# fengranMark/HAConvDR

Measured on AMD Instinct MI355X. Metric: queries/sec (encode+top-100) over N-passage 768-d corpus; HBM GB/s vs peak, higher is better.
Workload: dtype bf16 MFMA operands with fp32 accumulate / LayerNorm / softmax in the encoder (cosine vs the fp32 reference within 1e-3, measured ~1e-5); search scores and order = the fp32 fmaf chain, bit-exact

## Files before the change

haconvdr_amd/csrc/gemm8.inc:

```

enum { EPI8_QKV = 0, EPI8_RESID = 2, EPI8_GELU = 3 };
#ifndef G8_N1
#define G8_N1 4
#endif

struct Gemm8Args {
    const bf16 *A;
    const bf16 *W;
    int N, K;
    int n_groups;
    int n_tile0;
    const int *total_rows;
    const float2 *astats;
    const float *wsum;
    const float *cvec;
    bf16 *q, *k, *v16;
    const bf16 *resid;
    const float2 *rstats;
    const float *rgamma, *rbeta;
    bf16 *yb;
    float2 *part;
    bf16 *h;
    unsigned long long *clk;
    int stagger;
    int stagger_mode;
};

__device__ __forceinline__ void glds16(const bf16 *src, unsigned char *dst) {
    typedef const __attribute__((address_space(1))) void *gvp;
    typedef __attribute__((address_space(3))) void *lvp;
    __builtin_amdgcn_global_load_lds((gvp)src, (lvp)dst, 16, 0, 0);
}
__device__ __forceinline__ void swap16(unsigned &a, unsigned &b) {
    const auto r = __builtin_amdgcn_permlane16_swap(a, b, false, false);
    a = r[0];
    b = r[1];
}
__device__ __forceinline__ void quad_transpose4(f4v &v, int p) {
    int x0 = __float_as_int(v.x), x1 = __float_as_int(v.y), x2 = __float_as_int(v.z), x3 = __float_as_int(v.w);
    {
        const bool odd = p & 1;
        const int sa = odd ? x0 : x1, sb = odd ? x2 : x3;
        const int ra = __builtin_amdgcn_update_dpp(0, sa, 0xB1, 0xF, 0xF, false);
        const int rb = __builtin_amdgcn_update_dpp(0, sb, 0xB1, 0xF, 0xF, false);
        x0 = odd ? ra : x0;
        x1 = odd ? x1 : ra;
        x2 = odd ? rb : x2;
        x3 = odd ? x3 : rb;
    }
    {
        const bool hi = p & 2;
        const int sa = hi ? x0 : x2, sb = hi ? x1 : x3;
        const int ra = __builtin_amdgcn_update_dpp(0, sa, 0x4E, 0xF, 0xF, false);
        const int rb = __builtin_amdgcn_update_dpp(0, sb, 0x4E, 0xF, 0xF, false);
        x0 = hi ? ra : x0;
        x2 = hi ? x2 : ra;
        x1 = hi ? rb : x1;
        x3 = hi ? x3 : rb;
    }
    v.x = __int_as_float(x0);
    v.y = __int_as_float(x1);
    v.z = __int_as_float(x2);
    v.w = __int_as_float(x3);
}

__device__ __forceinline__ void xchg8(uint4 &a, uint4 &b, bool lo) {
    unsigned *pa = reinterpret_cast<unsigned *>(&a), *pb = reinterpret_cast<unsigned *>(&b);
#pragma unroll
    for (int i = 0; i < 4; ++i) {
        const unsigned send = lo ? pb[i] : pa[i];
        const unsigned recv = (unsigned)__builtin_amdgcn_update_dpp(0, (int)send, 0x128, 0xF, 0xF, false);
        pa[i] = lo ? pa[i] : recv;
        pb[i] = lo ? recv : pb[i];
    }
}

typedef unsigned g8_u4 __attribute__((ext_vector_type(4)));
typedef unsigned g8_u2 __attribute__((ext_vector_type(2)));
template <bool NT> __device__ __forceinline__ void g8_store16(void *p, uint4 v) {
    if constexpr (NT) __builtin_nontemporal_store(g8_u4{v.x, v.y, v.z, v.w}, reinterpret_cast<g8_u4 *>(p));
    else *reinterpret_cast<uint4 *>(p) = v;
}
template <bool NT> __device__ __forceinline__ void g8_store8(void *p, uint2 v) {
    if constexpr (NT) __builtin_nontemporal_store(g8_u2{v.x, v.y}, reinterpret_cast<g8_u2 *>(p));
    else *reinterpret_cast<uint2 *>(p) = v;
}

__device__ __forceinline__ unsigned pack_bf16(float lo, float hi) {
    typedef __bf16 bf16x2_t __attribute__((ext_vector_type(2)));
    bf16x2_t v;
    v.x = (bf16)lo;
    v.y = (bf16)hi;
    return __builtin_bit_cast(unsigned, v);
}

__device__ __forceinline__ f2v gelu8_2(f2v x) {
    f2v z = x * 0.70710678118654752f;
    z.x = __builtin_amdgcn_fmed3f(z.x, -3.0f, 3.0f);
    z.y = __builtin_amdgcn_fmed3f(z.y, -3.0f, 3.0f);
    const f2v u = z * z;
    f2v p = u * (-1.546677965e-07f) + 6.9032217e-06f;
    p = p * u + (-0.0001336812065f);
    p = p * u + 0.001487465865f;
    p = p * u + (-0.0106578986f);
    p = p * u + 0.0524059485f;
    p = p * u + (-0.1851637965f);
    p = p * u + 0.56346134f;
    return x * (z * p + 0.5f);
}

template <int EPI, bool NT>
__global__ __launch_bounds__(512, 2) void gemm8_kernel(Gemm8Args g) {
    extern __shared__ __attribute__((aligned(16))) unsigned char smem[];
    const int tid = threadIdx.x, lane = tid & 63;
    const int w = __builtin_amdgcn_readfirstlane(tid >> 6);
    const int wr = w >> 2, wc = w & 3;
    if constexpr (EPI == EPI8_GELU) {
        if (g.clk && blockIdx.x == 0 && tid == 0) {
            g.clk[0] = __builtin_amdgcn_s_memtime();
            g.clk[1] = __builtin_amdgcn_s_memrealtime();
        }
    }
    const int K = g.K, KT = K >> 6, nx = (g.N >> 8) - g.n_tile0;
    const int NG = g.n_groups, nxg = nx / NG, NP = 8 / NG;
    const int xcd = blockIdx.x & 7, slot = blockIdx.x >> 3, per_xcd = (gridDim.x + 7 - xcd) >> 3;
    const int mt_all = (*g.total_rows + 255) >> 8;
    const int mt_lo = (int)((long)mt_all * (xcd / NG) / NP), mt_hi = (int)((long)mt_all * (xcd / NG + 1) / NP);
    const int n_base = g.n_tile0 + (xcd % NG) * nxg;
    const int run_lo = 0, run_hi = (mt_hi - mt_lo) * nxg;
    const int tile0 = run_lo + slot;
    if (tile0 >= run_hi) return;
    const int my_tiles = (run_hi - tile0 + per_xcd - 1) / per_xcd;
    const int srow = lane >> 3;
    const int sch0 = (lane & 7) ^ (srow >> 1);
    const int chE = sch0 * 8, chO = (sch0 ^ 4) * 8;
    int s_tile = tile0, s_kt = 0;
    const bf16 *s_A = g.A + (size_t)((mt_lo + s_tile / nxg) << 8) * K, *s_W = g.W + (size_t)((n_base + s_tile % nxg) << 8) * K;
    const int wq = w & 3;
    const int so = EPI == EPI8_RESID ? wr : wr ^ 1;
    const unsigned lsrcE = (unsigned)(((so ? wq * 64 : wq * 32) + srow) * K + chE);
    const unsigned lsrcO = (unsigned)(((so ? wq * 64 : wq * 32) + 8 + srow) * K + chO);
    const int ring_base = (so ? 98304 : 0) + wq * 4096, ring_slots = so ? 4 : 6;
    int h_half = 0, h_slot = 0, h_p = 0;
    const bf16 *h_base = so ? s_W : s_A;
    long h_left = (long)my_tiles * KT * 8;
    constexpr int N1 = G8_N1, N2 = 8 - N1;
    auto issue_piece = [&]() __attribute__((always_inline)) {
        const bf16 *src = h_base + (size_t)(h_half * (so ? 32 : 128) + (h_p >> 1) * 16) * K + s_kt * 64;
        unsigned char *dst = smem + ring_base + (h_slot << 14) + h_p * 1024;
        glds16(src + ((h_p & 1) ? lsrcO : lsrcE), dst);
        if (++h_p == 4) {
            h_p = 0;
            h_slot = h_slot + 1 == ring_slots ? 0 : h_slot + 1;
            if (++h_half == 2) {
                h_half = 0;
                if (++s_kt == KT) {
                    s_kt = 0;
                    s_tile += per_xcd;
                    h_base = so ? g.W + (size_t)((n_base + s_tile % nxg) << 8) * K : g.A + (size_t)((mt_lo + s_tile / nxg) << 8) * K;
                }
            }
        }
    };
    auto issue_pieces = [&](auto ntag) __attribute__((always_inline)) -> bool {
        constexpr int n = decltype(ntag)::value;
        if (h_left <= 0) return false;
        h_left -= n;
#pragma unroll
        for (int i = 0; i < n; ++i) issue_piece();
        return true;
    };
    constexpr std::integral_constant<int, 16> n16tag{};
    constexpr std::integral_constant<int, 8> n8ktag{};

    const int m16 = lane & 15, kg = lane >> 4, sw = (m16 >> 1) & 7;
    const int c0 = ((kg ^ sw) << 4), c1 = (((4 + kg) ^ sw) << 4);
    const int a_row = (wr * 64 + m16) * 128, w_row = (wc * 32 + m16) * 128;

#ifdef G8_STAMP
    unsigned long long stamps[16] = {0, 0, 0, 0, 0, 0, 0, 0, 0, 0, 0, 0, 0, 0, 0, 0};
    unsigned long long est[16] = {0, 0, 0, 0, 0, 0, 0, 0, 0, 0, 0, 0, 0, 0, 0, 0};
#define G8_T(i, cond) if (cond) stamps[i] = __builtin_amdgcn_s_memtime()
#define G8_E(i) if (seq == 2) est[i] = __builtin_amdgcn_s_memtime()
#else
#define G8_E(i)
#define G8_T(i, cond)
#endif
#ifdef G8_STAMP2
    unsigned long long ph[16] = {0, 0, 0, 0, 0, 0, 0, 0, 0, 0, 0, 0, 0, 0, 0, 0};
#define G8_P(i) if (seq == 3 && kt == 6) ph[i] = __builtin_amdgcn_s_memtime()
#define G8_PM() if (seq == 3 && kt == 6) ph[5] = ph[6] = ph[13] = ph[7] = ph[8] = ph[9] = __builtin_amdgcn_s_memtime()
#else
#define G8_P(i)
#define G8_PM()
#endif
    constexpr bool RL = EPI == EPI8_RESID;
    f32x4 acc[2][2][4][2];
    bf16x8 wf0[2][2], wf1[2][2], af0[4][2];

    issue_pieces(n16tag);
    if (g.stagger) {
        const int ph = g.stagger_mode == 0 ? (xcd & 3) : g.stagger_mode == 1 ? (slot & 3) : g.stagger_mode == 2 ? xcd : (slot & 7);
        for (int i = ph * g.stagger; i > 0; --i) __builtin_amdgcn_s_sleep(32);
    }
    asm volatile("s_waitcnt vmcnt(0)" ::: "memory");
    __builtin_amdgcn_s_barrier();

    int a_cur = 0, w_cur = 0;
    for (int seq = 0; seq < my_tiles; ++seq) {
        const int tile = tile0 + seq * per_xcd;
        const int m0 = (mt_lo + tile / nxg) << 8, n0 = (n_base + tile % nxg) << 8;
        unsigned char *R1 = smem, *R2 = smem, *R3 = smem;
        const size_t rl_tb = (size_t)m0 * H + n0;
        auto rl_issue_sb = [&](int i, int mt, unsigned char *dst) __attribute__((always_inline)) {
            int ln = lane;
            asm volatile("" : "+v"(ln));
            const unsigned lo = (unsigned)((ln & 15) * H + (ln >> 5) * 16 + ((ln >> 4) & 1) * 8);
#if defined(G8_RL_ABL) && (G8_RL_ABL & 2)
            const bf16 *src = g.resid + (size_t)(wr * 64 + i * 128 + mt * 16) * H + wc * 64 + lo;
#else
            const bf16 *src = g.resid + (rl_tb + (size_t)(wr * 64 + i * 128 + mt * 16) * H + wc * 64) + lo;
#endif
            glds16(src, dst);
            glds16(src + 32, dst + 1024);
        };
        auto rl_issue_cols = [&](unsigned char *dst) __attribute__((always_inline)) {
            int ln = lane;
            asm volatile("" : "+v"(ln));
            const unsigned so = (unsigned)((ln >> 5) * 128 + 2 * (ln & 31));
            glds16(reinterpret_cast<const bf16 *>(g.rstats + ((size_t)m0 + wr * 64) + so), dst);
            const int sel = (ln >> 4) & 3;
            const float *pc = g.cvec, *pg = g.rgamma, *pb = g.rbeta;
            asm volatile("" : "+s"(pc), "+s"(pg), "+s"(pb));
            const float *vb = pc;
            vb = sel == 1 ? pg : vb;
            vb = sel == 2 ? pb : vb;
            glds16(reinterpret_cast<const bf16 *>(vb + (n0 + wc * 64) + 4 * (ln & 15)), dst + 1024);
        };
        G8_T(2, seq == 3);
        if (wr == 1) __builtin_amdgcn_s_barrier();
#pragma unroll
        for (int i = 0; i < 2; ++i)
#pragma unroll
            for (int j = 0; j < 2; ++j)
#pragma unroll
                for (int mt = 0; mt < 4; ++mt)
#pragma unroll
                    for (int nt = 0; nt < 2; ++nt)
#pragma unroll
                        for (int e = 0; e < 4; ++e) acc[i][j][mt][nt][e] = 0.f;

        for (int kt = 0; kt < KT; ++kt) {
            G8_P(0);
            const unsigned char *kbA = smem + a_cur * 32768, *kbW = smem + 98304 + w_cur * 32768;
            if constexpr (!RL) {
                const bool staged = (wr || kt) && issue_pieces(n8ktag);
                __builtin_amdgcn_sched_barrier(0);
                G8_P(12);
#pragma unroll
                for (int nt = 0; nt < 2; ++nt) {
                    wf0[nt][0] = *reinterpret_cast<const bf16x8 *>(kbW + w_row + nt * 2048 + c0);
                    wf0[nt][1] = *reinterpret_cast<const bf16x8 *>(kbW + w_row + nt * 2048 + c1);
                    wf1[nt][0] = *reinterpret_cast<const bf16x8 *>(kbW + 16384 + w_row + nt * 2048 + c0);
                    wf1[nt][1] = *reinterpret_cast<const bf16x8 *>(kbW + 16384 + w_row + nt * 2048 + c1);
                }
#pragma unroll
                for (int mt = 0; mt < 4; ++mt) {
                    af0[mt][0] = *reinterpret_cast<const bf16x8 *>(kbA + a_row + mt * 2048 + c0);
                    af0[mt][1] = *reinterpret_cast<const bf16x8 *>(kbA + a_row + mt * 2048 + c1);
                }
                __builtin_amdgcn_sched_barrier(0);
                G8_P(1);
                G8_P(2);
                if (wr && kt) {
                    if (staged) asm volatile("s_waitcnt vmcnt(8)" ::: "memory");
                    else asm volatile("s_waitcnt vmcnt(0)" ::: "memory");
                }
                asm volatile("s_waitcnt lgkmcnt(0)" ::: "memory");
                G8_P(3);
                __builtin_amdgcn_s_barrier();
                G8_P(4);
                G8_T(3 + (kt < 3 ? kt : 3), seq == 3 && kt < 4);
                __builtin_amdgcn_sched_barrier(0);
                __builtin_amdgcn_s_setprio(1);
                auto read_a1 = [&](auto mttag, auto kstag) __attribute__((always_inline)) {
                    constexpr int mt = decltype(mttag)::value, ks = decltype(kstag)::value;
                    __builtin_amdgcn_sched_barrier(0);
                    af0[mt][ks] = *reinterpret_cast<const bf16x8 *>(kbA + 16384 + a_row + mt * 2048 + (ks ? c1 : c0));
                    __builtin_amdgcn_sched_barrier(0);
                };
                constexpr std::integral_constant<int, 0> i0{};
                constexpr std::integral_constant<int, 1> i1{};
                constexpr std::integral_constant<int, 2> i2{};
                constexpr std::integral_constant<int, 3> i3{};
                auto mfma4 = [&](auto itag, auto mttag, auto kstag) __attribute__((always_inline)) {
                    constexpr int i = decltype(itag)::value, mt = decltype(mttag)::value, ks = decltype(kstag)::value;
#pragma unroll
                    for (int nt = 0; nt < 2; ++nt) {
                        acc[i][0][mt][nt] = __builtin_amdgcn_mfma_f32_16x16x32_bf16(wf0[nt][ks], af0[mt][ks], acc[i][0][mt][nt], 0, 0, 0);
                        acc[i][1][mt][nt] = __builtin_amdgcn_mfma_f32_16x16x32_bf16(wf1[nt][ks], af0[mt][ks], acc[i][1][mt][nt], 0, 0, 0);
                    }
                };
                mfma4(i0, i0, i0), read_a1(i0, i0);
                mfma4(i0, i1, i0), read_a1(i1, i0);
                mfma4(i0, i2, i0), read_a1(i2, i0);
                mfma4(i0, i3, i0), read_a1(i3, i0);
                mfma4(i0, i0, i1), read_a1(i0, i1);
                mfma4(i0, i1, i1), read_a1(i1, i1);
                mfma4(i0, i2, i1);
                mfma4(i0, i3, i1);
                __builtin_amdgcn_sched_barrier(0);
                G8_PM();
                mfma4(i1, i0, i0), read_a1(i2, i1);
                mfma4(i1, i1, i0), read_a1(i3, i1);
                mfma4(i1, i2, i0);
                mfma4(i1, i3, i0);
                __builtin_amdgcn_sched_barrier(0);
                mfma4(i1, i0, i1);
                mfma4(i1, i1, i1);
                mfma4(i1, i2, i1);
                mfma4(i1, i3, i1);
                __builtin_amdgcn_s_setprio(0);
                G8_P(10);
                if (wr == 0 && kt) asm volatile("s_waitcnt vmcnt(0)" ::: "memory");
                asm volatile("s_waitcnt lgkmcnt(0)" ::: "memory");
                __builtin_amdgcn_s_barrier();
                G8_P(11);
                a_cur = a_cur == 2 ? 0 : a_cur + 1;
                w_cur ^= 1;
                continue;
            }
            const bool lastk = RL && kt == KT - 1;
            const bool live1 = (wr == 0 || kt) && h_left > 0 && !(lastk && wr == 0);
            if (live1) {
                h_left -= N1;
#pragma unroll
                for (int i = 0; i < N1; ++i) issue_piece();
            }
            if constexpr (RL) {
                if (lastk) {
                    R1 = smem + (a_cur == 0 ? 2 : a_cur - 1) * 32768 + w * 4096;
                    R3 = smem + a_cur * 32768 + w * 4096;
                    R2 = smem + 98304 + w_cur * 32768 + w * 4096;
                    rl_issue_cols(R1);
                    rl_issue_sb(0, 0, R1 + 2048);
                }
            }
            __builtin_amdgcn_sched_barrier(0);
            G8_P(12);
#pragma unroll
            for (int nt = 0; nt < 2; ++nt) {
                wf0[nt][0] = *reinterpret_cast<const bf16x8 *>(kbW + w_row + nt * 2048 + c0);
                wf0[nt][1] = *reinterpret_cast<const bf16x8 *>(kbW + w_row + nt * 2048 + c1);
                wf1[nt][0] = *reinterpret_cast<const bf16x8 *>(kbW + 16384 + w_row + nt * 2048 + c0);
                wf1[nt][1] = *reinterpret_cast<const bf16x8 *>(kbW + 16384 + w_row + nt * 2048 + c1);
            }
#pragma unroll
            for (int mt = 0; mt < 4; ++mt) {
                af0[mt][0] = *reinterpret_cast<const bf16x8 *>(kbA + a_row + mt * 2048 + c0);
                af0[mt][1] = *reinterpret_cast<const bf16x8 *>(kbA + a_row + mt * 2048 + c1);
            }
            __builtin_amdgcn_sched_barrier(0);
            G8_P(1);
            G8_P(2);
            asm volatile("s_waitcnt lgkmcnt(0)" ::: "memory");
            G8_P(3);
            __builtin_amdgcn_s_barrier();
            G8_P(4);
            G8_T(3 + (kt < 3 ? kt : 3), seq == 3 && kt < 4);
            __builtin_amdgcn_sched_barrier(0);
            __builtin_amdgcn_s_setprio(1);
#pragma unroll
            for (int ks = 0; ks < 2; ++ks)
#pragma unroll
                for (int mt = 0; mt < 4; ++mt)
#pragma unroll
                    for (int nt = 0; nt < 2; ++nt) {
                        acc[0][0][mt][nt] = __builtin_amdgcn_mfma_f32_16x16x32_bf16(wf0[nt][ks], af0[mt][ks], acc[0][0][mt][nt], 0, 0, 0);
                        acc[0][1][mt][nt] = __builtin_amdgcn_mfma_f32_16x16x32_bf16(wf1[nt][ks], af0[mt][ks], acc[0][1][mt][nt], 0, 0, 0);
                    }
            __builtin_amdgcn_s_setprio(0);
            G8_P(5);
            __builtin_amdgcn_s_barrier();
            G8_P(6);
            const bool live2 = h_left > 0 && !lastk;
            if (live2) {
                h_left -= N2;
#pragma unroll
                for (int i = 0; i < N2; ++i) issue_piece();
            }
            if constexpr (RL) {
                if (lastk) {
                    rl_issue_sb(0, 1, R2);
                    rl_issue_sb(0, 2, R2 + 2048);
                }
            }
            __builtin_amdgcn_sched_barrier(0);
            G8_P(13);
#pragma unroll
            for (int mt = 0; mt < 4; ++mt) {
                af0[mt][0] = *reinterpret_cast<const bf16x8 *>(kbA + 16384 + a_row + mt * 2048 + c0);
                af0[mt][1] = *reinterpret_cast<const bf16x8 *>(kbA + 16384 + a_row + mt * 2048 + c1);
            }
            __builtin_amdgcn_sched_barrier(0);
            G8_P(7);
            if (lastk) {
            } else if (kt) {
                if (!live2) asm volatile("s_waitcnt vmcnt(0)" ::: "memory");
                else if (wr == 0) asm volatile("s_waitcnt vmcnt(8)" ::: "memory");
                else asm volatile("s_waitcnt vmcnt(%0)" ::"n"(N2) : "memory");
            }
            asm volatile("s_waitcnt lgkmcnt(0)" ::: "memory");
            G8_P(8);
            __builtin_amdgcn_s_barrier();
            G8_P(9);
            __builtin_amdgcn_sched_barrier(0);
            __builtin_amdgcn_s_setprio(1);
#pragma unroll
            for (int ks = 0; ks < 2; ++ks)
#pragma unroll
                for (int mt = 0; mt < 4; ++mt)
#pragma unroll
                    for (int nt = 0; nt < 2; ++nt) {
                        acc[1][0][mt][nt] = __builtin_amdgcn_mfma_f32_16x16x32_bf16(wf0[nt][ks], af0[mt][ks], acc[1][0][mt][nt], 0, 0, 0);
                        acc[1][1][mt][nt] = __builtin_amdgcn_mfma_f32_16x16x32_bf16(wf1[nt][ks], af0[mt][ks], acc[1][1][mt][nt], 0, 0, 0);
                    }
            __builtin_amdgcn_s_setprio(0);
            G8_P(10);
            __builtin_amdgcn_s_barrier();
            G8_P(11);
            a_cur = a_cur == 2 ? 0 : a_cur + 1;
            w_cur ^= 1;
        }
        G8_T(8, seq == 2 && true);
        if (wr == 0) __builtin_amdgcn_s_barrier();
        G8_T(0, seq == 2);
        if constexpr (!RL) {
            if (wr == 0) issue_pieces(n8ktag);
            asm volatile("s_waitcnt vmcnt(0)" ::: "memory");
        }
        G8_T(1, seq == 2);

#ifdef G8_NO_EPI
#pragma unroll
        for (int i = 0; i < 2; ++i)
#pragma unroll
            for (int j = 0; j < 2; ++j)
#pragma unroll
                for (int mt = 0; mt < 4; ++mt)
#pragma unroll
                    for (int nt = 0; nt < 2; ++nt) asm volatile("" ::"v"(acc[i][j][mt][nt]));
        continue;
#endif
        {
            const int colg = 8 * ((kg & 1) * 2 + (kg >> 1));
            if constexpr (RL) {
                const bool lo8 = m16 < 8;
                const unsigned lane_b = (unsigned)((wr * 64 + (m16 & 7)) * H + wc * 64 + (m16 >> 3) * 32 + colg);
                const unsigned rd_off = (unsigned)(((kg >> 1) * 16 + m16) * 16);
                const bool rd_hi = kg & 1;
#define G8_VM(n) asm volatile("s_waitcnt vmcnt(" #n ")" ::: "memory")
#define G8_VMC(c, a, b) do { if (c) G8_VM(a); else G8_VM(b); } while (0)
#define G8_LDS_DONE() asm volatile("s_waitcnt lgkmcnt(0)" ::: "memory")
                constexpr std::integral_constant<int, -1> cnone{};
                constexpr std::integral_constant<int, 0> c0t{};
                constexpr std::integral_constant<int, 1> c1t{};
                constexpr std::integral_constant<int, 2> c2t{};
                constexpr std::integral_constant<int, 3> c3t{};
                constexpr std::integral_constant<int, 8> n8tag{};
                rl_issue_sb(0, 3, R3);
                rl_issue_sb(1, 0, R3 + 2048);
                G8_E(0);
                G8_VM(8);
                G8_E(1);
                float mean_[2][4], rstd_[2][4];
                f4v rg[2][2], rb[2][2];
#pragma unroll
                for (int i = 0; i < 2; ++i)
#pragma unroll
                    for (int mt = 0; mt < 4; ++mt) {
                        g8_u4 c = *reinterpret_cast<const g8_u4 *>(R1 + i * 512 + (mt * 16 + (m16 & 14)) * 8);
                        asm volatile("" : "+v"(c));
                        asm volatile("v_mov_b32 %0, %1" : "=v"(mean_[i][mt]) : "v"((m16 & 1) ? c.z : c.x));
                        asm volatile("v_mov_b32 %0, %1" : "=v"(rstd_[i][mt]) : "v"((m16 & 1) ? c.w : c.y));
                    }
#pragma unroll
                for (int jj = 0; jj < 2; ++jj)
#pragma unroll
                    for (int nt = 0; nt < 2; ++nt) {
                        const int co = (jj * 32 + nt * 16 + 4 * kg) * 4;
                        const f4v cvv = *reinterpret_cast<const f4v *>(R1 + 1024 + co);
#pragma unroll
                        for (int i = 0; i < 2; ++i)
#pragma unroll
                            for (int mt = 0; mt < 4; ++mt) acc[i][jj][mt][nt] += cvv;
                        rg[jj][nt] = *reinterpret_cast<const f4v *>(R1 + 1024 + 256 + co);
                        rb[jj][nt] = *reinterpret_cast<const f4v *>(R1 + 1024 + 512 + co);
                    }
                auto sb_read = [&](const unsigned char *sb, g8_u4 (&c)[2][2]) __attribute__((always_inline)) {
#pragma unroll
                    for (int jj = 0; jj < 2; ++jj) {
                        c[jj][0] = *reinterpret_cast<const g8_u4 *>(sb + jj * 1024 + rd_off);
                        c[jj][1] = *reinterpret_cast<const g8_u4 *>(sb + jj * 1024 + 512 + rd_off);
                        asm volatile("" : "+v"(c[jj][0]), "+v"(c[jj][1]));
                    }
                };
                auto sb_do = [&](auto itag, auto mttag, unsigned char *sb, auto refilltag, const g8_u4 (*pre)[2]) __attribute__((always_inline)) {
                    constexpr int i = decltype(itag)::value, mt = decltype(mttag)::value, refill = decltype(refilltag)::value;
                    const float mean = mean_[i][mt], rstd = rstd_[i][mt];
                    uint4 ro[2];
                    float s1 = 0.f, s2 = 0.f;
                    g8_u4 cc[2][2];
                    if (pre) {
#pragma unroll
                        for (int jj = 0; jj < 2; ++jj) cc[jj][0] = pre[jj][0], cc[jj][1] = pre[jj][1];
                    } else {
                        sb_read(sb, cc);
                    }
#pragma unroll
                    for (int jj = 0; jj < 2; ++jj) {
                        const g8_u4 c0 = cc[jj][0], c1 = cc[jj][1];
                        const uint2 w0 = {rd_hi ? c0.z : c0.x, rd_hi ? c0.w : c0.y}, w1 = {rd_hi ? c1.z : c1.x, rd_hi ? c1.w : c1.y};
                        const f4v ra = {__uint_as_float(w0.x << 16), __uint_as_float(w0.x & 0xffff0000u), __uint_as_float(w0.y << 16), __uint_as_float(w0.y & 0xffff0000u)};
                        const f4v rb_ = {__uint_as_float(w1.x << 16), __uint_as_float(w1.x & 0xffff0000u), __uint_as_float(w1.y << 16), __uint_as_float(w1.y & 0xffff0000u)};
                        const f4v o0 = acc[i][jj][mt][0] + ((ra - mean) * rstd * rg[jj][0] + rb[jj][0]);
                        const f4v o1 = acc[i][jj][mt][1] + ((rb_ - mean) * rstd * rg[jj][1] + rb[jj][1]);
                        unsigned p0 = pack_bf16(o0.x, o0.y), p1 = pack_bf16(o0.z, o0.w);
                        unsigned p2 = pack_bf16(o1.x, o1.y), p3 = pack_bf16(o1.z, o1.w);
                        swap16(p0, p2);
                        swap16(p1, p3);
                        ro[jj] = make_uint4(p0, p1, p2, p3);
                        const f4v sm = o0 + o1, sq = o0 * o0 + o1 * o1;
                        const float t1 = (sm.x + sm.y) + (sm.z + sm.w), t2 = (sq.x + sq.y) + (sq.z + sq.w);
                        s1 = jj ? s1 + t1 : t1;
                        s2 = jj ? s2 + t2 : t2;
                    }
                    s1 += __shfl_xor(s1, 16);
                    s2 += __shfl_xor(s2, 16);
                    s1 += __shfl_xor(s1, 32);
                    s2 += __shfl_xor(s2, 32);
                    xchg8(ro[0], ro[1], lo8);
                    G8_LDS_DONE();
                    if constexpr (refill >= 0) rl_issue_sb(1, refill, sb);
                    __builtin_amdgcn_sched_barrier(0);
                    const size_t row = (size_t)m0 + i * 128 + wr * 64 + mt * 16 + m16;
#if defined(G8_RL_ABL) && (G8_RL_ABL & 1)
                    if (lane == 0) g.part[row * (g.N >> 6) + (n0 >> 6) + wc] = make_float2(s1, s2);
#pragma unroll
                    for (int jj = 0; jj < 2; ++jj)
                        if (lane == 0) g8_store16<NT>(g.yb + rl_tb + (size_t)((i * 128 + mt * 16 + jj * 8) * H) + lane_b, ro[jj]);
#else
                    if (kg == 0) g.part[row * (g.N >> 6) + (n0 >> 6) + wc] = make_float2(s1, s2);
#pragma unroll
                    for (int jj = 0; jj < 2; ++jj)
                        g8_store16<NT>(g.yb + rl_tb + (size_t)((i * 128 + mt * 16 + jj * 8) * H) + lane_b, ro[jj]);
#endif
                    __builtin_amdgcn_sched_barrier(0);
                };
                __builtin_amdgcn_sched_barrier(0);
                bool gA = false, gW = false;
                sb_do(c0t, c0t, R1 + 2048, cnone, nullptr);
                G8_E(2);
                __builtin_amdgcn_s_barrier();
                if (wr == 0) gA = issue_pieces(n8tag);
                __builtin_amdgcn_sched_barrier(0);
                G8_E(3);
                G8_VMC(gA, 17, 9);
                G8_E(4);
                sb_do(c0t, c1t, R2, c1t, nullptr);
                G8_VMC(gA, 20, 12);
                G8_E(5);
                sb_do(c0t, c2t, R2 + 2048, c2t, nullptr);
                G8_VMC(gA, 23, 15);
                G8_E(6);
                sb_do(c0t, c3t, R3, c3t, nullptr);
                G8_VMC(gA, 26, 18);
                G8_E(7);
                sb_do(c1t, c0t, R3 + 2048, cnone, nullptr);
                G8_VM(16);
                G8_E(8);
                sb_do(c1t, c1t, R2, cnone, nullptr);
                G8_VM(14);
                G8_E(9);
                sb_do(c1t, c2t, R2 + 2048, cnone, nullptr);
                G8_E(10);
                G8_VM(12);
                G8_E(11);
                g8_u4 c7[2][2];
                sb_read(R3, c7);
                G8_LDS_DONE();
                __builtin_amdgcn_s_barrier();
                if (wr == 1) gW = issue_pieces(n8tag);
                __builtin_amdgcn_sched_barrier(0);
                G8_E(12);
                sb_do(c1t, c3t, R3, cnone, c7);
                G8_E(13);
                G8_VMC(gW, 3, 27);
                G8_E(14);
                G8_E(15);
#undef G8_VM
#undef G8_VMC
#undef G8_LDS_DONE
            } else {
                float2 st[2][4];
#pragma unroll
                for (int i = 0; i < 2; ++i)
#pragma unroll
                    for (int mt = 0; mt < 4; ++mt) st[i][mt] = g.astats[(size_t)m0 + i * 128 + wr * 64 + mt * 16 + m16];
                const int ldo = EPI == EPI8_GELU ? g.N : H;
                const bool lo8 = m16 < 8;
                const unsigned lane_b = (unsigned)((wr * 64 + (m16 & 7)) * ldo + wc * 64 + (m16 >> 3) * 32 + colg);
                f4v ws[2][2], cv[2][2];
#pragma unroll
                for (int j = 0; j < 2; ++j)
#pragma unroll
                    for (int nt = 0; nt < 2; ++nt) {
                        const int nb = n0 + wc * 64 + j * 32;
                        cv[j][nt] = *reinterpret_cast<const f4v *>(g.cvec + nb + nt * 16 + 4 * kg);
                        ws[j][nt] = *reinterpret_cast<const f4v *>(g.wsum + nb + nt * 16 + 4 * kg);
                    }
#pragma unroll
                for (int i = 0; i < 2; ++i)
#pragma unroll
                    for (int mt = 0; mt < 4; ++mt) {
                        const float nm = -st[i][mt].x * st[i][mt].y;
                        float rs = st[i][mt].y;
                        asm volatile("v_mov_b32 %0, %1" : "=v"(rs) : "v"(st[i][mt].y));
                        uint4 o[2];
#pragma unroll
                        for (int j = 0; j < 2; ++j) {
                            const int nb = n0 + wc * 64 + j * 32;
                            unsigned p[4];
#pragma unroll
                            for (int nt = 0; nt < 2; ++nt) {
                                f4v v = acc[i][j][mt][nt] * rs + (ws[j][nt] * nm + cv[j][nt]);
                                if (EPI == EPI8_QKV && n0 >= 2 * H) {
                                    quad_transpose4(v, lane & 3);
                                    const int n = nb + nt * 16 + 4 * kg + (lane & 3) - 2 * H;
                                    const size_t mg = (size_t)(m0 + i * 128 + wr * 64 + mt * 16) >> 4;
                                    uint2 o2;
                                    o2.x = pack_bf16(v.x, v.y);
                                    o2.y = pack_bf16(v.z, v.w);
                                    g8_store8<NT>(g.v16 + (mg * H + n) * 16 + (m16 & 12), o2);
                                    continue;
                                }
                                if constexpr (EPI == EPI8_GELU) {
                                    const f2v g0 = gelu8_2((f2v){v.x, v.y}), g1 = gelu8_2((f2v){v.z, v.w});
                                    p[2 * nt] = pack_bf16(g0.x, g0.y);
                                    p[2 * nt + 1] = pack_bf16(g1.x, g1.y);
                                } else {
                                    p[2 * nt] = pack_bf16(v.x, v.y);
                                    p[2 * nt + 1] = pack_bf16(v.z, v.w);
                                }
                            }
                            if (EPI == EPI8_QKV && n0 >= 2 * H) continue;
                            swap16(p[0], p[2]);
                            swap16(p[1], p[3]);
                            o[j] = make_uint4(p[0], p[1], p[2], p[3]);
                        }
                        if (EPI == EPI8_QKV && n0 >= 2 * H) continue;
                        xchg8(o[0], o[1], lo8);
                        const size_t ur = (size_t)(m0 + i * 128 + mt * 16) * ldo;
#pragma unroll
                        for (int j = 0; j < 2; ++j) {
                            if constexpr (EPI == EPI8_GELU) {
                                g8_store16<NT>(g.h + ur + (size_t)(j * 8) * ldo + n0 + lane_b, o[j]);
                            } else {
                                bf16 *dst = n0 < H ? g.q + ur + n0 : g.k + ur + (n0 - H);
                                g8_store16<NT>(dst + (size_t)(j * 8) * ldo + lane_b, o[j]);
                            }
                        }
                    }
            }
        }
    }
    if constexpr (EPI == EPI8_GELU) {
        if (g.clk && blockIdx.x == 0 && tid == 0) {
            g.clk[2] = __builtin_amdgcn_s_memtime();
            g.clk[3] = __builtin_amdgcn_s_memrealtime();
        }
    }
#ifdef G8_STAMP2
    if (blockIdx.x == 8 && lane == 0 && (w == 0 || w == 4)) {
        unsigned long long *o = reinterpret_cast<unsigned long long *>(g.part) + 64 + (w ? 16 : 0);
        for (int i = 0; i < 16; ++i) o[i] = ph[i];
    }
#endif
#ifdef G8_STAMP
    if (blockIdx.x == 8 && lane == 0 && (w == 0 || w == 4)) {
        unsigned long long *o = reinterpret_cast<unsigned long long *>(g.part) + (w ? 16 : 0);
        for (int i = 0; i < 16; ++i) o[i] = stamps[i];
        for (int i = 0; i < 16; ++i) o[32 + i] = est[i];
    }
#endif
}

__global__ __launch_bounds__(256) void ln_combine_kernel(const float2 *__restrict__ part, int n_part, int n_cols, const int *__restrict__ total_rows,
                                                         float eps, float2 *__restrict__ stats) {
    const size_t row = (size_t)blockIdx.x * 256 + threadIdx.x;
    if (row >= (size_t)((*total_rows + 255) & ~255)) return;
    float s1 = 0.f, s2 = 0.f;
    if ((n_part & 1) == 0) {
        const float4 *p4 = reinterpret_cast<const float4 *>(part + row * n_part);
        float4 v[8];
        const int n4 = n_part >> 1;
#pragma unroll
        for (int i = 0; i < 8; ++i) v[i] = i < n4 ? p4[i] : make_float4(0.f, 0.f, 0.f, 0.f);
#pragma unroll
        for (int i = 0; i < 8; ++i) {
            s1 += v[i].x + v[i].z;
            s2 += v[i].y + v[i].w;
        }
        for (int i = 16; i < n_part; ++i) {
            const float2 p = part[row * n_part + i];
            s1 += p.x;
            s2 += p.y;
        }
    } else {
        for (int i = 0; i < n_part; ++i) {
            const float2 p = part[row * n_part + i];
            s1 += p.x;
            s2 += p.y;
        }
    }
    const float mean = s1 / n_cols;
    const float var = fmaxf(s2 / n_cols - mean * mean, 0.f);
    stats[row] = make_float2(mean, rsqrtf(var + eps));
}

__global__ __launch_bounds__(256) void fold_ln_kernel(const float *__restrict__ Wf, const float *__restrict__ bias, const float *__restrict__ gamma,
                                                      const float *__restrict__ beta, int K, float scale, bf16 *__restrict__ Wb,
                                                      float *__restrict__ wsum, float *__restrict__ cvec) {
    __shared__ float red[2][4];
    const int n = blockIdx.x, tid = threadIdx.x;
    float s = 0.f, c = 0.f;
    for (int k = tid; k < K; k += 256) {
        const float wv = Wf[(size_t)n * K + k];
        const bf16 wb = (bf16)(wv * (gamma ? gamma[k] : 1.f) * scale);
        Wb[(size_t)n * K + k] = wb;
        s += (float)wb;
        if (beta) c += beta[k] * wv;
    }
    s = wave_sum(s);
    c = wave_sum(c);
    if ((tid & 63) == 0) {
        red[0][tid >> 6] = s;
        red[1][tid >> 6] = c;
    }
    __syncthreads();
    if (tid == 0) {
        wsum[n] = gamma ? (red[0][0] + red[0][1]) + (red[0][2] + red[0][3]) : 0.f;
        cvec[n] = (bias[n] + (red[1][0] + red[1][1]) + (red[1][2] + red[1][3])) * scale;
    }
}

__global__ void fill_identity_stats_kernel(float2 *__restrict__ stats, size_t n) {
    const size_t i = (size_t)blockIdx.x * blockDim.x + threadIdx.x;
    if (i < n) stats[i] = make_float2(0.f, 1.f);
}
```

Measured before the change: 8192.

## Swap A/W operand roles for V tiles to drop the quad-transpose epilogue

For QKV tiles in the V range, the loader now swaps which half of the ring receives A and which receives W. The MFMA result therefore comes out already transposed, and the V epilogue can store the transposed bf16 layout directly. This removes the DPP quad_transpose4 shuffles and the scattered 8-byte stores. The per-row stats and wsum/cvec are now loaded along the opposite axes. It also adds timestamp probe macros. The risk is correctness of the role swap and the new index math.

```diff
diff --git a/haconvdr_amd/csrc/gemm8.inc b/haconvdr_amd/csrc/gemm8.inc
--- a/haconvdr_amd/csrc/gemm8.inc
+++ b/haconvdr_amd/csrc/gemm8.inc
@@ -36,34 +36,6 @@
     a = r[0];
     b = r[1];
 }
-__device__ __forceinline__ void quad_transpose4(f4v &v, int p) {
-    int x0 = __float_as_int(v.x), x1 = __float_as_int(v.y), x2 = __float_as_int(v.z), x3 = __float_as_int(v.w);
-    {
-        const bool odd = p & 1;
-        const int sa = odd ? x0 : x1, sb = odd ? x2 : x3;
-        const int ra = __builtin_amdgcn_update_dpp(0, sa, 0xB1, 0xF, 0xF, false);
-        const int rb = __builtin_amdgcn_update_dpp(0, sb, 0xB1, 0xF, 0xF, false);
-        x0 = odd ? ra : x0;
-        x1 = odd ? x1 : ra;
-        x2 = odd ? rb : x2;
-        x3 = odd ? x3 : rb;
-    }
-    {
-        const bool hi = p & 2;
-        const int sa = hi ? x0 : x2, sb = hi ? x1 : x3;
-        const int ra = __builtin_amdgcn_update_dpp(0, sa, 0x4E, 0xF, 0xF, false);
-        const int rb = __builtin_amdgcn_update_dpp(0, sb, 0x4E, 0xF, 0xF, false);
-        x0 = hi ? ra : x0;
-        x2 = hi ? x2 : ra;
-        x1 = hi ? rb : x1;
-        x3 = hi ? x3 : rb;
-    }
-    v.x = __int_as_float(x0);
-    v.y = __int_as_float(x1);
-    v.z = __int_as_float(x2);
-    v.w = __int_as_float(x3);
-}
-
 __device__ __forceinline__ void xchg8(uint4 &a, uint4 &b, bool lo) {
     unsigned *pa = reinterpret_cast<unsigned *>(&a), *pb = reinterpret_cast<unsigned *>(&b);
 #pragma unroll
@@ -143,6 +115,12 @@
     const int ring_base = (so ? 98304 : 0) + wq * 4096, ring_slots = so ? 4 : 6;
     int h_half = 0, h_slot = 0, h_p = 0;
     const bf16 *h_base = so ? s_W : s_A;
+    auto swapped_base = [&](int t) __attribute__((always_inline)) -> const bf16 * {
+        const int nt_ = n_base + t % nxg, mt_ = mt_lo + t / nxg;
+        const bool vt = (nt_ << 8) >= 2 * H;
+        return (so != 0) != vt ? g.W + (size_t)(nt_ << 8) * K : g.A + (size_t)(mt_ << 8) * K;
+    };
+    if constexpr (EPI == EPI8_QKV) h_base = swapped_base(s_tile);
     long h_left = (long)my_tiles * KT * 8;
     constexpr int N1 = G8_N1, N2 = 8 - N1;
     auto issue_piece = [&]() __attribute__((always_inline)) {
@@ -157,7 +135,8 @@
                 if (++s_kt == KT) {
                     s_kt = 0;
                     s_tile += per_xcd;
-                    h_base = so ? g.W + (size_t)((n_base + s_tile % nxg) << 8) * K : g.A + (size_t)((mt_lo + s_tile / nxg) << 8) * K;
+                    if constexpr (EPI == EPI8_QKV) h_base = swapped_base(s_tile);
+                    else h_base = so ? g.W + (size_t)((n_base + s_tile % nxg) << 8) * K : g.A + (size_t)((mt_lo + s_tile / nxg) << 8) * K;
                 }
             }
         }
@@ -182,8 +161,10 @@
     unsigned long long est[16] = {0, 0, 0, 0, 0, 0, 0, 0, 0, 0, 0, 0, 0, 0, 0, 0};
 #define G8_T(i, cond) if (cond) stamps[i] = __builtin_amdgcn_s_memtime()
 #define G8_E(i) if (seq == 2) est[i] = __builtin_amdgcn_s_memtime()
+#define G8_V(i, cond) if (cond) est[i] = __builtin_amdgcn_s_memtime()
 #else
 #define G8_E(i)
+#define G8_V(i, cond)
 #define G8_T(i, cond)
 #endif
 #ifdef G8_STAMP2
@@ -281,6 +262,7 @@
                 __builtin_amdgcn_s_barrier();
                 G8_P(4);
                 G8_T(3 + (kt < 3 ? kt : 3), seq == 3 && kt < 4);
+                G8_V(4, seq == 4 && kt == 0);
                 __builtin_amdgcn_sched_barrier(0);
                 __builtin_amdgcn_s_setprio(1);
                 auto read_a1 = [&](auto mttag, auto kstag) __attribute__((always_inline)) {
@@ -602,6 +584,63 @@
 #undef G8_VMC
 #undef G8_LDS_DONE
             } else {
+                if constexpr (EPI == EPI8_QKV) {
+                    if (n0 >= 2 * H) {
+                        G8_V(2, seq == 3);
+                        f4v rs[2][2], nm[2][2];
+                        float wsf[2][4], cvf[2][4];
+                        float4 sab[2][2][2];
+#pragma unroll
+                        for (int j = 0; j < 2; ++j)
+#pragma unroll
+                            for (int nt = 0; nt < 2; ++nt) {
+                                const float4 *sp = reinterpret_cast<const float4 *>(g.astats + ((size_t)m0 + wc * 64 + j * 32 + nt * 16 + 4 * kg));
+                                sab[j][nt][0] = sp[0];
+                                sab[j][nt][1] = sp[1];
+                            }
+#pragma unroll
+                        for (int i = 0; i < 2; ++i)
+#pragma unroll
+                            for (int mt = 0; mt < 4; ++mt) {
+                                const int n = n0 + i * 128 + wr * 64 + mt * 16 + m16;
+                                wsf[i][mt] = g.wsum[n];
+                                cvf[i][mt] = g.cvec[n];
+                            }
+                        __builtin_amdgcn_sched_barrier(0);
+#pragma unroll
+                        for (int j = 0; j < 2; ++j)
+#pragma unroll
+                            for (int nt = 0; nt < 2; ++nt) {
+                                const float4 sa = sab[j][nt][0], sb = sab[j][nt][1];
+                                float r0, r1, r2, r3;
+                                asm volatile("v_mov_b32 %0, %1" : "=v"(r0) : "v"(sa.y));
+                                asm volatile("v_mov_b32 %0, %1" : "=v"(r1) : "v"(sa.w));
+                                asm volatile("v_mov_b32 %0, %1" : "=v"(r2) : "v"(sb.y));
+                                asm volatile("v_mov_b32 %0, %1" : "=v"(r3) : "v"(sb.w));
+                                rs[j][nt] = (f4v){r0, r1, r2, r3};
+                                nm[j][nt] = (f4v){-sa.x * sa.y, -sa.z * sa.w, -sb.x * sb.y, -sb.z * sb.w};
+                            }
+                        bf16 *vb = g.v16 + ((size_t)((m0 + wc * 64) >> 4) * H + (n0 - 2 * H)) * 16;
+                        const unsigned lane_v = (unsigned)((wr * 64 + m16) * 16 + 4 * kg);
+#pragma unroll
+                        for (int i = 0; i < 2; ++i)
+#pragma unroll
+                            for (int mt = 0; mt < 4; ++mt)
+#pragma unroll
+                                for (int j = 0; j < 2; ++j)
+#pragma unroll
+                                    for (int nt = 0; nt < 2; ++nt) {
+                                        const f4v v = acc[i][j][mt][nt] * rs[j][nt] + (nm[j][nt] * wsf[i][mt] + cvf[i][mt]);
+                                        uint2 o2;
+                                        o2.x = pack_bf16(v.x, v.y);
+                                        o2.y = pack_bf16(v.z, v.w);
+                                        g8_store8<NT>(vb + (size_t)((j * 2 + nt) * H + i * 128 + mt * 16) * 16 + lane_v, o2);
+                                    }
+                        G8_V(3, seq == 3);
+                        continue;
+                    }
+                }
+                G8_V(0, seq == 2);
                 float2 st[2][4];
 #pragma unroll
                 for (int i = 0; i < 2; ++i)
@@ -629,21 +668,10 @@
                         uint4 o[2];
 #pragma unroll
                         for (int j = 0; j < 2; ++j) {
-                            const int nb = n0 + wc * 64 + j * 32;
                             unsigned p[4];
 #pragma unroll
                             for (int nt = 0; nt < 2; ++nt) {
                                 f4v v = acc[i][j][mt][nt] * rs + (ws[j][nt] * nm + cv[j][nt]);
-                                if (EPI == EPI8_QKV && n0 >= 2 * H) {
-                                    quad_transpose4(v, lane & 3);
-                                    const int n = nb + nt * 16 + 4 * kg + (lane & 3) - 2 * H;
-                                    const size_t mg = (size_t)(m0 + i * 128 + wr * 64 + mt * 16) >> 4;
-                                    uint2 o2;
-                                    o2.x = pack_bf16(v.x, v.y);
-                                    o2.y = pack_bf16(v.z, v.w);
-                                    g8_store8<NT>(g.v16 + (mg * H + n) * 16 + (m16 & 12), o2);
-                                    continue;
-                                }
                                 if constexpr (EPI == EPI8_GELU) {
                                     const f2v g0 = gelu8_2((f2v){v.x, v.y}), g1 = gelu8_2((f2v){v.z, v.w});
                                     p[2 * nt] = pack_bf16(g0.x, g0.y);
@@ -653,12 +681,10 @@
                                     p[2 * nt + 1] = pack_bf16(v.z, v.w);
                                 }
                             }
-                            if (EPI == EPI8_QKV && n0 >= 2 * H) continue;
                             swap16(p[0], p[2]);
                             swap16(p[1], p[3]);
                             o[j] = make_uint4(p[0], p[1], p[2], p[3]);
                         }
-                        if (EPI == EPI8_QKV && n0 >= 2 * H) continue;
                         xchg8(o[0], o[1], lo8);
                         const size_t ur = (size_t)(m0 + i * 128 + mt * 16) * ldo;
 #pragma unroll
@@ -671,6 +697,7 @@
                             }
                         }
                     }
+                G8_V(1, seq == 2);
             }
         }
     }
```

Result: no change. 8263, median of 6 (+0.9%).
